# CloudResolvingClimateModeling/sp-coupler

Measured on AMD Instinct MI355X. Metric: SP column-exchanges/sec (GCM<->LES forcing+tendency), higher is better.
Workload: dtype f64

## Files before the change

sp_coupler_amd/csrc/spc_hip.hip:

```cpp
#include <hip/hip_runtime.h>
#include <stdint.h>
#include <stdio.h>
#include <stdlib.h>
#include <string.h>

#include <initializer_list>
#include <type_traits>
#include <unordered_map>

#include "spc.h"

#pragma clang fp contract(off)

#include "spc_pow_coefs.h"
__constant__ double spc_pow_coef_table[21] = {SPC_POW_COEFS};
#define SPC_POW_TABLE spc_pow_coef_table

#ifndef SPC_MUTANT
#define SPC_MUTANT 0
#endif
#define SPC_MUT(n, mutated, original) (SPC_MUTANT == (n) ? (mutated) : (original))

namespace {

// ... 157 lines not shown
template <typename T> struct Bracket {
    int j;
    int mode;
    T x, x0, x1;
};

template <typename T> __device__ __forceinline__ Bracket<T> bracket(const T *xp, int n, int p2, T x)
{
    Bracket<T> b;
    b.x = x;
    if (n == 1) { b.mode = 1; b.j = 0; b.x0 = b.x1 = x; return b; }
    if (x != x) { b.mode = 2; b.j = 0; b.x0 = b.x1 = x; return b; }
    const int j = upper_count(xp, n, p2, x) - 1;
    if (j < 0) { b.mode = 1; b.j = 0; b.x0 = b.x1 = x; return b; }
    if (j >= n - 1) { b.mode = 1; b.j = n - 1; b.x0 = b.x1 = x; return b; }
    b.j = j;
    b.x0 = xp[j];
    b.x1 = xp[j + 1];
    b.mode = (b.x0 == x) ? 1 : 0;
    return b;
}

template <typename T> __device__ __forceinline__ T interp_at(const Bracket<T> &b, const T *fp)
{
    if (b.mode == 2) return b.x;
    if (b.mode == 1) return fp[b.j];
    return lerp_np(b.x, b.x0, b.x1, fp[b.j], fp[b.j + 1]);
}

template <typename T> struct Br {
    int j0, j1;
    bool take, nanx;
    T x, x0, x1;
};

template <typename T> __device__ __forceinline__ Br<T> bracket2(const T *xp, int n, int p2, T x)
{
    Br<T> b;
    const int j = upper_count(xp, n, p2, x) - 1;
    const bool below = j < 0, above = j >= n - 1;
    const int jmax = n >= 2 ? n - 2 : 0;
    const int jc = j < 0 ? 0 : (j > jmax ? jmax : j);
    const T x0 = xp[jc], x1 = xp[jc + 1 < n ? jc + 1 : n - 1];
    b.take = (n == 1) | below | above | (x0 == x);
    b.nanx = (x != x) & (n != 1);
    b.j0 = above ? n - 1 : jc;
    b.j1 = b.take ? b.j0 : jc + 1;
    b.x = x;
    b.x0 = b.take ? T(0) : x0;
    b.x1 = b.take ? T(1) : x1;
    return b;
}

template <int NF, typename T> __device__ __forceinline__ void interp_fields(const Br<T> &b, const T (&f0)[NF], const T (&f1)[NF], T (&r)[NF])
{
    const T t0 = b.x - b.x0;
    const Divisor<T> dx(b.x1 - b.x0);
    T slope[NF];
    bool any_nan = false;
#pragma unroll
    for (int k = 0; k < NF; ++k) {
        slope[k] = dx.div(f1[k] - f0[k]);
        r[k] = slope[k] * t0 + f0[k];
        any_nan |= (r[k] != r[k]);
    }
    if (any_nan & !b.take & !b.nanx) {
        const T t1 = b.x - b.x1;
#pragma unroll
        for (int k = 0; k < NF; ++k) {
            if (r[k] != r[k]) {
                T q = slope[k] * t1 + f1[k];
                if (q != q && f0[k] == f1[k]) q = f0[k];
                r[k] = q;
            }
        }
    }
#pragma unroll
    for (int k = 0; k < NF; ++k) r[k] = b.nanx ? b.x : (b.take ? f0[k] : r[k]);
}

struct DimsP {
    int64_t n_cols, pitchG, pitchGh, pitchL;
    int nG, nL, cb, p2G, p2L, shared_grid, xcd_remap;
};

struct Empty {};

template <typename T> struct FwdOpt {
    const T *rain, *rain_last;
    T *u, *v, *thl, *qt, *ps, *Zf, *Zh, *rainrate;
    const T *Z0M, *Z0H, *QLflux, *QIflux, *SHflux, *TSflux;
    T *z0m, *z0h, *wthl, *wqt;
};

template <typename T, bool FULL> struct FwdP {
    DimsP d;
    const T *U, *V, *Tm, *SH, *QL, *QI, *Pf, *Ph, *Zgfull, *Zghalf, *zf, *zh;
    const T *u_d, *v_d, *thl_d, *qt_d, *ql_d, *ps_d;
    T factor, dt;
    T *f_u, *f_v, *f_thl, *f_qt, *f_ql, *ql_ref, *f_ps;
    int32_t *idx;
    typename std::conditional<FULL, FwdOpt<T>, Empty>::type o;
};

template <typename T> using FwdFull = FwdP<T, true>;

template <typename T> struct BwdP {
    DimsP d;
    const T *Tm, *SH, *QL, *QI, *U, *V, *A, *Zf, *Zgfull, *Zghalf, *zf;
    const T *t_d, *qt_d, *ql_d, *ql_ice_d, *u_d, *v_d, *A_prof;
    const T *zh, *Zh, *rhobf_d;
    T factor, dt;
    T *f_T, *f_SH, *f_QL, *f_QI, *f_U, *f_V, *f_A;
    int32_t *start_index;
};

template <typename T> struct DiagP {
    DimsP d;
    const T *Tm, *SH, *QL, *QI, *Pf, *Zgfull, *Zghalf, *zf, *thl_d, *ql_d, *ql_ice_d;
    T *Tv, *THL, *QT, *Zf, *Zh, *pf, *t, *ql_water;
};

extern __shared__ __align__(16) unsigned char spc_smem[];

__device__ __forceinline__ unsigned slab_index(int remap)
{
    if (remap) {
        const unsigned b = blockIdx.x, nb = gridDim.x, x = b & 7u, j = b >> 3, q = nb >> 3, r = nb & 7u;
        return x * q + (x < r ? x : r) + j;
    }
    return blockIdx.x;
}

#ifdef SPC_STAMPS
__device__ unsigned long long *g_stamps = nullptr;
#define STAMP(i)                                                                     \
    do {                                                                             \
        if (threadIdx.x == 0 && g_stamps && (SPC_STAMPS == 1 || (i) == 0 || (i) == 5)) {  \
            asm volatile("s_waitcnt vmcnt(0) lgkmcnt(0)" ::: "memory");              \
            g_stamps[(size_t)blockIdx.x * 8 + (i)] = wall_clock64();                 \
        }                                                                            \
    } while (0)
#else
#define STAMP(i) do { } while (0)
#endif

template <typename T> struct LesIn {
    T h, ud, vd, thld, qtd, qld;
};

template <typename P, typename T = decltype(+*P().zf)>
__device__ __forceinline__ LesIn<T> load_les(const P &p, int l, int64_t o)
{
    LesIn<T> r;
    r.h = p.d.shared_grid ? ldg(&p.zf[l]) : ldg(&p.zf[o]);
    r.ud = ldg(&p.u_d[o]); r.vd = ldg(&p.v_d[o]); r.thld = ldg(&p.thl_d[o]); r.qtd = ldg(&p.qt_d[o]); r.qld = ldg(&p.ql_d[o]);
    return r;
}

constexpr int cfloor_pow2(int n) { int p = 1; while (p * 2 <= n) p *= 2; return p; }

template <typename T, bool FULL, int NG, int NL, int WT, int BLK = BLOCK, bool PRE = true>
__global__ __launch_bounds__(BLK) void k_forward(const FwdP<T, FULL> p)
{
    const DimsP &d = p.d;
#define OPT(f) (*(decltype(FwdOpt<T>::f) const volatile __attribute__((address_space(4))) *)( \
// ... 142 lines not shown
                f0[k] = s[(k + 1) * nG + b.j0];
                f1[k] = s[(k + 1) * nG + b.j1];
            }
            interp_fields<5>(b, f0, f1, r);
            const T thl = r[0], qt = r[1], ql = r[2], u = r[3], v = r[4];
            stg<WT>(&p.f_u[o], ddt.div(p.factor * (u - SPC_MUT(2, in.vd, in.ud))));
            stg<WT>(&p.f_v[o], ddt.div(p.factor * (v - SPC_MUT(2, in.ud, in.vd))));
            stg<WT>(&p.f_thl[o], ddt.div(p.factor * (thl - in.thld)));
            stg<WT>(&p.f_qt[o], ddt.div(p.factor * (qt - in.qtd)));
            stg<WT>(&p.f_ql[o], ddt.div(p.factor * (ql - in.qld)));
            stg<WT>(&p.ql_ref[o], ql);
            if constexpr (FULL) {
                if (OPT(u)) OPT(u)[o] = u;
                if (OPT(v)) OPT(v)[o] = v;
                if (OPT(thl)) OPT(thl)[o] = thl;
                if (OPT(qt)) OPT(qt)[o] = qt;
            }
        } else {
            const int ei = e - n2, c = ei / nG, m = ei - c * nG;
            const int64_t col = col0 + c, gh = col * pitchGh;
            const T zgh = (PRE && e == tid) ? pre_zgh : ldg(&p.Zghalf[gh + (nG - 1 - m)]);
            const T zs = (PRE && e == tid) ? pre_zs : ldg(&p.Zghalf[gh + nG]);
            const T Zh_k = div_grav(zgh - zs);
            const T *const zh = d.shared_grid ? lzh : lzh + (size_t)c * nL;
            p.idx[col * pitchG + m] = SPC_MUT(5, ss_left_pos(zh, nL, Zh_k), ss_right(zh, nL, Zh_k));
        }
    }
    STAMP(4);

    if constexpr (FULL) {
        if (OPT(Zh)) {
            for (int e = tid; e < ncol * (nG + 1); e += BLK) {
                const int c = e / (nG + 1), k = e - c * (nG + 1);
                const int64_t gh = (col0 + c) * pitchGh;
                OPT(Zh)[gh + k] = div_grav(ldg(&p.Zghalf[gh + k]) - ldg(&p.Zghalf[gh + nG]));
            }
        }
    }
    STAMP(5);
#undef OPT
}

template <typename T>
__global__ __launch_bounds__(BLOCK) void k_cloud_idx(const DimsP d, const T *zh_, const T *Zh_, int32_t *idx)
{
    const int nG = d.nG, nL = d.nL, cb = d.cb, tid = threadIdx.x;
    const int64_t col0 = (int64_t)slab_index(d.xcd_remap) * cb;
    const int ncol = (int)((d.n_cols - col0) < cb ? (d.n_cols - col0) : cb);
    T *const lzh = reinterpret_cast<T *>(spc_smem);
    const int nz = d.shared_grid ? nL : ncol * nL;
    for (int e = tid; e < nz; e += BLOCK) {
        const int c = e / nL, l = e - c * nL;
        lzh[e] = d.shared_grid ? zh_[e] : zh_[(col0 + c) * d.pitchL + l];
    }
    __syncthreads();
    for (int e = tid; e < ncol * nG; e += BLOCK) {
        const int c = e / nG, m = e - c * nG;
        const int64_t col = col0 + c;
        const T *const zh = d.shared_grid ? lzh : lzh + (size_t)c * nL;
        idx[col * d.pitchG + m] = ss_right(zh, nL, Zh_[col * d.pitchGh + (nG - 1 - m)]);
    }
}

template <typename T> struct GcmIn {
    T tt, sh, ql, qi, u, v, a, a_d;
};

template <typename T> __device__ __forceinline__ GcmIn<T> load_gcm(const BwdP<T> &p, int64_t g, int64_t g_rev)
{
    GcmIn<T> r;
    r.tt = ldg(&p.Tm[g]); r.sh = ldg(&p.SH[g]); r.ql = ldg(&p.QL[g]); r.qi = ldg(&p.QI[g]); r.u = ldg(&p.U[g]); r.v = ldg(&p.V[g]); r.a = ldg(&p.A[g]);
    r.a_d = ldg(&p.A_prof[g_rev]);
    return r;
}

template <typename T, int NG, int NL, int WT, int BLK = BLOCK, bool PRE = true> __global__ __launch_bounds__(BLK) void k_backward(const BwdP<T> p)
{
    const DimsP &d = p.d;
    const int nG = NG ? NG : d.nG, nL = NL ? NL : d.nL, cb = d.cb, tid = threadIdx.x;
    const int64_t pitchG = NG ? NG : d.pitchG, pitchGh = NG ? NG + 1 : d.pitchGh, pitchL = NL ? NL : d.pitchL;
    const int p2L = NL ? cfloor_pow2(NL ? NL : 1) : d.p2L;
    const int64_t col0 = (int64_t)slab_index(d.xcd_remap) * cb;
    const int ncol = (int)((d.n_cols - col0) < cb ? (d.n_cols - col0) : cb);
    const size_t per_col = (size_t)6 * nL + nG;
    T *const lds = reinterpret_cast<T *>(spc_smem);
    T *const lh = lds + (size_t)cb * per_col;
    const int n1 = ncol * nG;
    STAMP(0);

    struct Stage { T t, qt, ql, qi, u, v, h; };
    auto load_stage = [&](int64_t o) {
        Stage r;
        r.t = ldg(&p.t_d[o]); r.qt = ldg(&p.qt_d[o]); r.ql = ldg(&p.ql_d[o]); r.qi = ldg(&p.ql_ice_d[o]);
        r.u = ldg(&p.u_d[o]); r.v = ldg(&p.v_d[o]);
        r.h = d.shared_grid ? T(0) : ldg(&p.zf[o]);
        return r;
    };
    auto load_zf = [&](int64_t col, int64_t g) {
        return p.Zf ? p.Zf[g] : div_grav(ldg(&p.Zgfull[g]) - ldg(&p.Zghalf[col * pitchGh + nG]));
    };
    const int n2 = ncol * nL;
    Stage st0 = {};
    T zf0 = T(0), hs0 = T(0);
    if (tid < n2) {
        const int c = tid / nL, l = tid - c * nL;
        st0 = load_stage((col0 + c) * pitchL + l);
    }
    if (tid < n1) {
        const int c = tid / nG, k = tid - c * nG;
        zf0 = load_zf(col0 + c, (col0 + c) * pitchG + k);
    }
    if (d.shared_grid && tid < nL) hs0 = ldg(&p.zf[tid]);
    GcmIn<T> pre = {};
    if (PRE && tid < n1) {
        const int c = tid / nG, k = tid - c * nG;
        const int64_t cg = (col0 + c) * pitchG;
        pre = load_gcm(p, cg + k, SPC_MUT(9, (col0 + ((c ^ 1) < ncol ? (c ^ 1) : c)) * pitchG, cg) + (nG - 1 - k));
    }
    STAMP(1);

    constexpr int UF = sizeof(T) == 4 ? 2 : 1;
    for (int e0 = tid; e0 < n2; e0 += UF * BLK) {
        Stage st[UF];
#pragma unroll
        for (int u = 0; u < UF; ++u) {
            const int e = e0 + u * BLK;
            if (e < n2) {
                const int c = e / nL, l = e - c * nL;
                st[u] = (e == tid) ? st0 : load_stage((col0 + c) * pitchL + l);
            }
        }
#pragma unroll
        for (int u = 0; u < UF; ++u) {
            const int e = e0 + u * BLK;
            if (e < n2) {
                const int c = e / nL, l = e - c * nL;
                T *const s = lds + (size_t)c * per_col + l;
                s[0] = st[u].t;
                s[nL] = st[u].qt;
                s[2 * nL] = st[u].ql;
                s[3 * nL] = st[u].qi;
                s[4 * nL] = st[u].u;
                s[5 * nL] = st[u].v;
                if (!d.shared_grid) lh[e] = st[u].h;
            }
        }
    }
    if (d.shared_grid)
        for (int e = tid; e < nL; e += BLK) lh[e] = (e == tid) ? hs0 : ldg(&p.zf[e]);
    for (int e = tid; e < n1; e += BLK) {
        const int c = e / nG, k = e - c * nG;
        const int64_t col = col0 + c;
        lds[(size_t)c * per_col + 6 * nL + k] = (e == tid) ? zf0 : load_zf(col, col * pitchG + k);
    }
    STAMP(2);
    __syncthreads();
    STAMP(3);

    const Divisor<T> ddt(p.dt);
    auto gcm_item = [&](int e, const GcmIn<T> &in) {
        const int c = e / nG, k = e - c * nG;
        const int64_t col = col0 + c, cg = col * pitchG, g = cg + k;
        const T *const s = lds + (size_t)c * per_col;
        const T *const h = d.shared_grid ? lh : lh + (size_t)c * nL;
        const T *const Zf = s + 6 * nL;
        const T x = Zf[k];
        const int start_index = ss_left_neg(Zf, nG, h[nL - 1]);
        const Bracket<T> b = bracket(h, nL, p2L, x);
        T t_i, qt_i, ql_i, qlw_i, qli_i, u_i, v_i;
        if (b.mode == 0) {
            const int j = b.j;
            const T ql0 = s[2 * nL + j], ql1 = s[2 * nL + j + 1], qi0 = s[3 * nL + j], qi1 = s[3 * nL + j + 1];
            const Divisor<T> dx(b.x1 - b.x0);
            t_i = lerp_np(x, b.x0, b.x1, s[j], s[j + 1], dx);
            qt_i = lerp_np(x, b.x0, b.x1, s[nL + j], s[nL + j + 1], dx);
            ql_i = lerp_np(x, b.x0, b.x1, ql0, ql1, dx);
            qlw_i = lerp_np(x, b.x0, b.x1, ql0 - qi0, ql1 - qi1, dx);
            qli_i = lerp_np(x, b.x0, b.x1, qi0, qi1, dx);
            u_i = lerp_np(x, b.x0, b.x1, s[4 * nL + j], s[4 * nL + j + 1], dx);
            v_i = lerp_np(x, b.x0, b.x1, s[5 * nL + j], s[5 * nL + j + 1], dx);
        } else if (b.mode == 1) {
            const int j = b.j;
            t_i = s[j];
            qt_i = s[nL + j];
            ql_i = s[2 * nL + j];
            qli_i = s[3 * nL + j];
            qlw_i = ql_i - qli_i;
            u_i = s[4 * nL + j];
            v_i = s[5 * nL + j];
        } else {
            t_i = qt_i = ql_i = qlw_i = qli_i = u_i = v_i = x;
        }
        T f_T = ddt.div(p.factor * SPC_MUT(24, in.tt - t_i, t_i - in.tt));
        T f_SH = ddt.div(p.factor * (SPC_MUT(13, qt_i, qt_i - ql_i) - in.sh));
        T f_QL = ddt.div(p.factor * (SPC_MUT(3, ql_i, qlw_i) - in.ql));
        T f_QI = ddt.div(p.factor * (qli_i - in.qi));
        T f_U = ddt.div(p.factor * (SPC_MUT(22, v_i, u_i) - in.u));
        T f_V = ddt.div(p.factor * (v_i - in.v));
        T f_A = ddt.div(p.factor * (in.a_d - in.a));
        if (SPC_MUT(4, k <= start_index, k < start_index)) {
            const T zero = T(0);
            f_T *= zero; f_SH *= zero; f_QL *= zero; f_QI *= zero; f_U *= zero; f_V *= zero; f_A *= zero;
        }
        stg<WT>(&p.f_T[g], f_T);
        stg<WT>(&p.f_SH[g], f_SH);
        stg<WT>(&p.f_QL[g], f_QL);
        stg<WT>(&p.f_QI[g], f_QI);
        stg<WT>(&p.f_U[g], f_U);
        stg<WT>(&p.f_V[g], f_V);
        stg<WT>(&p.f_A[g], f_A);
        if (p.start_index && k == 0) p.start_index[col] = start_index;
    };
    for (int e0 = tid; e0 < n1; e0 += UF * BLK) {
        GcmIn<T> in[UF];
#pragma unroll
        for (int u = 0; u < UF; ++u) {
            const int e = e0 + u * BLK;
            if (e < n1) {
                const int c = e / nG, k = e - c * nG;
                const int64_t cg = (col0 + c) * pitchG;
                in[u] = (PRE && e == tid) ? pre
                                          : load_gcm(p, cg + k, SPC_MUT(9, (col0 + ((c ^ 1) < ncol ? (c ^ 1) : c)) * pitchG, cg) + (nG - 1 - k));
            }
        }
#pragma unroll
        for (int u = 0; u < UF; ++u)
            if (e0 + u * BLK < n1) gcm_item(e0 + u * BLK, in[u]);
    }
    STAMP(4);
    STAMP(5);
}

#include "spc_f32v.hpp"
#include "spc_vnudge.hpp"
#include "spc_vnudge2.hpp"

template <typename T> __device__ __forceinline__ int scan_cell(const T *z, int n, T a)
{
    int lo = 1, hi = n - 1;
    while (lo < hi) {
        const int mid = lo + ((hi - lo) >> 1);
        if (z[mid] < a) lo = mid + 1; else hi = mid;
    }
    return lo - 1;
}

__host__ __device__ inline int su_pad(int p2) { return 2 * p2 + 2; }

template <int SL, typename T, typename Pred> __device__ __forceinline__ const T *su_seek(const T *row, int p2, const Pred &adv)
{
    const T *p = row;
    if constexpr (SL > 0) {
#pragma unroll
        for (int s = 1 << (SL - 1); s > 0; s >>= 1) {
            const T *const nx = p + s;
            p = adv(p[s - 1]) ? nx : p;
        }
    } else {
        for (int s = p2; s > 0; s >>= 1) {
            const T *const nx = p + s;
            p = adv(p[s - 1]) ? nx : p;
        }
    }
    return p;
}

template <int SL, typename T, typename Pred> __device__ __forceinline__ int su_count(const T *row, int p2, const Pred &adv)
{
    return (int)(((unsigned)(size_t)su_seek<SL>(row, p2, adv) - (unsigned)(size_t)row) / (unsigned)sizeof(T));
}

#include "spc_k4.hpp"
// ... 124 lines not shown
    thread_local int cache[64] = {0};
    int dev = 0;
    if (hipGetDevice(&dev) != hipSuccess) {
        (void)hipGetLastError();
        return 256;
    }
    if (dev >= 0 && dev < 64 && cache[dev]) return cache[dev];
    int n = 0;
    if (hipDeviceGetAttribute(&n, hipDeviceAttributeMultiprocessorCount, dev) != hipSuccess || n <= 0) {
        (void)hipGetLastError();
        n = 256;
    }
    if (dev >= 0 && dev < 64) cache[dev] = n;
    return n;
}

template <typename KernelT> int blocks_per_cu(KernelT kernel, size_t smem)
{
    thread_local std::unordered_map<uint64_t, int> cache;
    const uint64_t key = (uint64_t)(uintptr_t)kernel * 1000003u + smem;
    auto it = cache.find(key);
    if (it != cache.end()) return it->second;
    int nb = 0;
    if (hipOccupancyMaxActiveBlocksPerMultiprocessor(&nb, kernel, BLOCK, smem) != hipSuccess || nb <= 0) {
        (void)hipGetLastError();
        const size_t by_lds = smem ? (size_t)(160 * 1024) / smem : 8;
        nb = (int)(by_lds < 4 ? by_lds : 4);
    }
    if (nb > 8) nb = 8;
    cache[key] = nb;
    return nb;
}

template <typename KernelT> int pick_cb(const spc_dims *d, int pass, bool with_idx, size_t esize, KernelT kernel)
{
    size_t per_col, fixed;
    lds_elems(d, pass, with_idx, &per_col, &fixed, esize);
    int cb = d->cols_per_block;
    if (cb > 0) {
        while (cb > 1 && (per_col * cb + fixed) * esize > (size_t)MAX_LDS_BYTES) --cb;
        return cb;
    }
    int nb[4] = {0, 0, 0, 0};
    const int64_t cus = device_cus();
    for (int i = 0; i < 4; ++i) {
        cb = 1 << i;
        const size_t smem = (per_col * cb + fixed) * esize;
        if (cb > 1 && smem > (size_t)MAX_LDS_BYTES) continue;
        nb[i] = blocks_per_cu(kernel, smem);
        if (cb <= 4 && (d->n_cols + cb - 1) / cb <= cus * nb[i]) return cb;
    }
    if (pass == 4 && nb[1] * 2 > nb[0] && (d->n_cols + 1) / 2 >= 2 * cus * nb[1]) return 2;
    int best = 1, best_nb = -1;
    for (int i = (pass == 1 && esize == 4) ? 1 : 3; i >= 0; --i) {
        cb = 1 << i;
        const int64_t rounds_x_cus = nb[i] ? (d->n_cols + cb - 1) / cb / nb[i] : 0;
        const bool enough = rounds_x_cus >= (cb == 8 ? 8 : 2) * cus;
        if (nb[i] > best_nb && (enough || i == 0)) { best_nb = nb[i]; best = cb; }
    }
    return best;
}

int small_batch(int64_t bytes_written, int limit_mib = 32)
{
    return bytes_written <= (int64_t)limit_mib * 1024 * 1024 ? 1 : 0;
}

int geometry_id(const spc_dims *d)
{
    if (d->pitchG != d->nG || d->pitchGh != d->nG + 1 || d->pitchL != d->nL) return 0;
    if (d->nG == 91 && d->nL == 160) return 1;
    if (d->nG == 137 && d->nL == 512) return 2;
    if (d->nG == 19 && d->nL == 160) return 3;
    return 0;
}

DimsP make_dims(const spc_dims *d, int cb)
{
    DimsP p;
    p.n_cols = d->n_cols; p.pitchG = d->pitchG; p.pitchGh = d->pitchGh; p.pitchL = d->pitchL;
    p.nG = d->nG; p.nL = d->nL; p.cb = cb; p.p2G = floor_pow2(d->nG); p.p2L = floor_pow2(d->nL);
    p.shared_grid = d->les_grid_shared != 0;
    p.xcd_remap = cb <= 2;
    return p;
}

template <typename KernelT> int ensure_lds(KernelT kernel, size_t smem, const char *what)
{
    if (smem <= (size_t)MAX_LDS_BYTES) return SPC_OK;
    if (smem > (size_t)HARD_LDS_BYTES)
        return fail(SPC_ERR_UNSUPPORTED, "%s needs %lld B of LDS per workgroup (gfx950 has %lld)", what, (long long)smem, HARD_LDS_BYTES);
    if (hipFuncSetAttribute(reinterpret_cast<const void *>(kernel), hipFuncAttributeMaxDynamicSharedMemorySize, (int)smem) != hipSuccess) {
        (void)hipGetLastError();
        return fail(SPC_ERR_UNSUPPORTED, "%s: cannot raise the dynamic LDS limit to %lld B", what, (long long)smem);
    }
    return SPC_OK;
}

int launch_status(const char *what)
{
    const hipError_t e = hipGetLastError();
    if (e == hipSuccess) return SPC_OK;
    snprintf(g_err, sizeof(g_err), "%s: %s", what, hipGetErrorString(e));
    return SPC_ERR_LAUNCH;
}

#define REQUIRE(ptr, name) \
    if (!(ptr)) return fail(SPC_ERR_INVALID_ARGUMENT, "required pointer %s is NULL", name)

int small_block(const spc_dims *d, int items_per_col)
{
    const int64_t cus = device_cus();
    if (d->cols_per_block != 0 || items_per_col > BLOCK || d->n_cols <= cus || d->n_cols > 4 * cus) return 0;
    const int sb = env_int("SPC_SMALL_BLOCK", 1);
    if (!sb) return 0;
    if (sb == 2 || sb == 4) return sb;
    return d->n_cols <= 2 * cus ? 2 : 4;
}

struct Choice {
    const char *kernel;
    int elem, full, idx, geo, wt, blk, pre, cb;
    int vec = 0;
    unsigned grid;
    size_t smem;
};

constexpr int GEO_NG[4] = {0, 91, 137, 19}, GEO_NL[4] = {0, 160, 512, 160};

template <typename T> using KLean = void (*)(const FwdP<T, false>);
template <typename T> using KFull = void (*)(const FwdP<T, true>);
template <typename T> using KBwd = void (*)(const BwdP<T>);

#define SPC_FWD_ROW(FULL_, WT_, BLK_, PRE_)                                                                          \
    {k_forward<T, FULL_, 0, 0, WT_, BLK_, PRE_>, k_forward<T, FULL_, 91, 160, WT_, BLK_, PRE_>,                      \
     k_forward<T, FULL_, 137, 512, WT_, BLK_, PRE_>, k_forward<T, FULL_, 19, 160, WT_, BLK_, PRE_>}
#define SPC_FWD_ROW_BIG(BLK_)                                                                                        \
    {k_forward<T, false, 0, 0, 1, BLK_, true>, k_forward<T, false, 91, 160, 1, BLK_, true>, nullptr,                 \
     k_forward<T, false, 19, 160, 1, BLK_, true>}

template <typename T> KLean<T> fwd_lean_kernel(int geo, int wt, int blk, int pre)
{
    static const KLean<T> k256[2][2][4] = {{SPC_FWD_ROW(false, 0, BLOCK, false), SPC_FWD_ROW(false, 1, BLOCK, false)},
                                           {SPC_FWD_ROW(false, 0, BLOCK, true), SPC_FWD_ROW(false, 1, BLOCK, true)}};
    static const KLean<T> k512[4] = SPC_FWD_ROW_BIG(512), k1024[4] = SPC_FWD_ROW_BIG(1024);
    if (blk == BLOCK) return k256[pre][wt][geo];
    if (!wt || !pre) return nullptr;
    return blk == 512 ? k512[geo] : (blk == 1024 ? k1024[geo] : nullptr);
}

template <typename T> KFull<T> fwd_full_kernel(int geo, int pre)
{
    static const KFull<T> k[2][4] = {SPC_FWD_ROW(true, 0, BLOCK, false), SPC_FWD_ROW(true, 0, BLOCK, true)};
    return k[pre][geo];
}
#undef SPC_FWD_ROW
#undef SPC_FWD_ROW_BIG

template <typename T> int choose_fwd(const spc_dims *d, bool with_idx, bool full, Choice *c)
{
    c->kernel = "k_forward"; c->elem = (int)sizeof(T); c->full = full; c->idx = with_idx;
    c->geo = geometry_id(d);
    c->wt = full ? 0 : small_batch(d->n_cols * (int64_t)((6 * d->nL + 1) * sizeof(T) + (with_idx ? d->nG * 4 : 0)));
    const int sb = (full || !c->wt) ? 0 : small_block(d, d->nL + (with_idx ? d->nG : 0));
    const int pre_env = env_int("SPC_K1_PRE", -1);
    c->pre = (sb || (pre_env >= 0 ? pre_env != 0 : d->n_cols <= 4 * (int64_t)device_cus())) ? 1 : 0;
    c->blk = sb ? BLOCK * sb : BLOCK;
    if (full)
        c->cb = pick_cb(d, 0, with_idx, sizeof(T), fwd_full_kernel<T>(c->geo, c->pre));
    else
        c->cb = sb ? sb : pick_cb(d, 0, with_idx, sizeof(T), fwd_lean_kernel<T>(c->geo, 0, BLOCK, c->pre));
    size_t per_col, fixed;
    lds_elems(d, 0, with_idx, &per_col, &fixed);
    c->smem = (per_col * c->cb + fixed) * sizeof(T);
    c->grid = (unsigned)((d->n_cols + c->cb - 1) / c->cb);
    c->vec = std::is_same<T, float>::value && c->geo != 0 && !full && !sb && !c->pre && c->cb % 2 == 0 && env_int("SPC_F32_VEC", 1);
    return SPC_OK;
}

inline KLean<float> fwd_vec_kernel(int geo, int wt)
{
    static const KLean<float> k[2][4] = {{nullptr, k_forward_f32v<91, 160, 0>, k_forward_f32v<137, 512, 0>, k_forward_f32v<19, 160, 0>},
                                         {nullptr, k_forward_f32v<91, 160, 1>, k_forward_f32v<137, 512, 1>, k_forward_f32v<19, 160, 1>}};
    return k[wt ? 1 : 0][geo];
}
inline bool aligned8(std::initializer_list<const void *> ptrs)
{
    for (const void *q : ptrs) if ((uintptr_t)q & 7u) return false;
    return true;
}

template <typename T> int forward_impl(const spc_dims *d, const spc_forward_args *a, void *stream)
{
    int rc = validate(d);
    if (rc) return rc;
    if (!a) return fail(SPC_ERR_INVALID_ARGUMENT, "%sargs is NULL");
    if (d->n_cols == 0) return SPC_OK;
    REQUIRE(a->U, "U"); REQUIRE(a->V, "V"); REQUIRE(a->T, "T"); REQUIRE(a->SH, "SH"); REQUIRE(a->QL, "QL");
    REQUIRE(a->QI, "QI"); REQUIRE(a->Pf, "Pf"); REQUIRE(a->Ph, "Ph"); REQUIRE(a->Zgfull, "Zgfull");
    REQUIRE(a->Zghalf, "Zghalf"); REQUIRE(a->zf, "zf"); REQUIRE(a->u_d, "u_d"); REQUIRE(a->v_d, "v_d");
    REQUIRE(a->thl_d, "thl_d"); REQUIRE(a->qt_d, "qt_d"); REQUIRE(a->ql_d, "ql_d"); REQUIRE(a->ps_d, "ps_d");
    REQUIRE(a->f_u, "f_u"); REQUIRE(a->f_v, "f_v"); REQUIRE(a->f_thl, "f_thl"); REQUIRE(a->f_qt, "f_qt");
    REQUIRE(a->f_ql, "f_ql"); REQUIRE(a->ql_ref, "ql_ref"); REQUIRE(a->f_ps, "f_ps");
    if (a->idx && !a->zh) return fail(SPC_ERR_INVALID_ARGUMENT, "%sidx requested but zh is NULL");
    if (a->rainrate && (!a->rain || !a->rain_last))
        return fail(SPC_ERR_INVALID_ARGUMENT, "%srainrate requested but rain / rain_last is NULL");
// ... 48 lines not shown
    int rc = validate(d);
    if (rc) return rc;
    if (d->n_cols == 0) return SPC_OK;
    REQUIRE(zh, "zh"); REQUIRE(Zh, "Zh"); REQUIRE(idx, "idx");
    const int cb = pick_cb(d, 2, true, sizeof(T), k_cloud_idx<T>);
    size_t per_col, fixed;
    lds_elems(d, 2, true, &per_col, &fixed);
    const size_t smem = (per_col * cb + fixed) * sizeof(T);
    if ((rc = ensure_lds(k_cloud_idx<T>, smem, "cloud_indices"))) return rc;
    const unsigned grid = (unsigned)((d->n_cols + cb - 1) / cb);
    hipLaunchKernelGGL(k_cloud_idx<T>, dim3(grid), dim3(BLOCK), smem, (hipStream_t)stream, make_dims(d, cb),
                       (const T *)zh, (const T *)Zh, idx);
    return launch_status("k_cloud_idx");
}

#define SPC_BWD_ROW(WT_, BLK_, PRE_)                                                                                 \
    {k_backward<T, 0, 0, WT_, BLK_, PRE_>, k_backward<T, 91, 160, WT_, BLK_, PRE_>, k_backward<T, 137, 512, WT_, BLK_, PRE_>, \
     k_backward<T, 19, 160, WT_, BLK_, PRE_>}
#define SPC_BWD_ROW_BIG(BLK_)                                                                                        \
    {k_backward<T, 0, 0, 1, BLK_, true>, k_backward<T, 91, 160, 1, BLK_, true>, nullptr, k_backward<T, 19, 160, 1, BLK_, true>}

template <typename T> KBwd<T> bwd_kernel(int geo, int wt, int blk, int pre)
{
    static const KBwd<T> k256[2][2][4] = {{SPC_BWD_ROW(0, BLOCK, false), SPC_BWD_ROW(1, BLOCK, false)},
                                          {SPC_BWD_ROW(0, BLOCK, true), SPC_BWD_ROW(1, BLOCK, true)}};
    static const KBwd<T> k512[4] = SPC_BWD_ROW_BIG(512), k1024[4] = SPC_BWD_ROW_BIG(1024);
    if (blk == BLOCK) return k256[pre][wt][geo];
    if (!wt || !pre) return nullptr;
    return blk == 512 ? k512[geo] : (blk == 1024 ? k1024[geo] : nullptr);
}
#undef SPC_BWD_ROW
#undef SPC_BWD_ROW_BIG

template <typename T> KBwd<T> cons_kernel(int geo, int pd, int cb)
{
    static const KBwd<T> k3[4][2] = {{nullptr, nullptr},
                                     {k_backward_cons3<T, 91, 160, 1>, k_backward_cons3<T, 91, 160, 2>},
                                     {k_backward_cons3<T, 137, 512, 1>, k_backward_cons3<T, 137, 512, 2>},
                                     {k_backward_cons3<T, 19, 160, 1>, k_backward_cons3<T, 19, 160, 2>}};
    if (geo != 0) return k3[geo][cb >= 2 ? 1 : 0];
    if constexpr (std::is_same<T, double>::value) {
        static const KBwd<T> kd[3] = {k_backward_cons2<T, 0, 0, 1>, k_backward_cons2<T, 0, 0, 2>, k_backward_cons2<T, 0, 0, 3>};
        if (pd >= 1 && pd <= 3) return kd[pd - 1];
    }
    return k_backward_cons2<T, 0, 0, -1>;
}

template <typename T> int pick_cb_cons3(const spc_dims *d, int geo)
{
    size_t per_col, fixed;
    lds_elems(d, 4, false, &per_col, &fixed, sizeof(T));
    const size_t smem1 = (per_col + fixed) * sizeof(T), smem2 = (2 * per_col + fixed) * sizeof(T);
    const bool two_fits = smem2 <= (size_t)MAX_LDS_BYTES;
    if (d->cols_per_block > 0) return (d->cols_per_block >= 2 && two_fits) ? 2 : 1;
    const int nb1 = blocks_per_cu(cons_kernel<T>(geo, 0, 1), smem1);
    if (d->n_cols <= (int64_t)device_cus() * nb1 || !two_fits) return 1;
    const int nb2 = blocks_per_cu(cons_kernel<T>(geo, 0, 2), smem2);
    return nb2 * 2 > nb1 ? 2 : 1;
}

int cons_depth(int nL)
{
    if (nL > 1024) return -1;
    static const struct Tab { signed char d[1025]; Tab() { int m = 0; for (int n = 0; n <= 1024; ++n) { if (n >= 129) { const int dn = vn_pw_depth_of(n); if (dn > m) m = dn; } d[n] = (signed char)m; } } } tab;
    const int d = nL < 0 ? 0 : tab.d[nL];
    return d < 1 ? 1 : (d <= 3 ? d : -1);
}

template <typename T> int choose_bwd(const spc_dims *d, bool cons, Choice *c)
{
    c->kernel = cons ? "k_backward_cons2" : "k_backward"; c->elem = (int)sizeof(T); c->full = cons; c->idx = 0;
    c->geo = geometry_id(d);
    c->wt = cons ? 0 : small_batch(d->n_cols * (int64_t)(7 * d->nG * sizeof(T)), 14);
    const int sb = (cons || !c->wt) ? 0 : small_block(d, d->nL > d->nG ? d->nL : d->nG);
    const int64_t cus = device_cus();
    c->pre = (cons || sb || d->n_cols <= 4 * cus || d->n_cols * 256 > 25000 * cus) ? 1 : 0;
    c->blk = sb ? BLOCK * sb : BLOCK;
    c->cb = sb ? sb : (cons ? (c->geo ? pick_cb_cons3<T>(d, c->geo) : pick_cb(d, 4, false, sizeof(T), cons_kernel<T>(0, cons_depth(d->nL), 0)))
                            : pick_cb(d, 1, false, sizeof(T), bwd_kernel<T>(c->geo, 0, BLOCK, c->pre)));
    size_t per_col, fixed;
    lds_elems(d, cons ? 4 : 1, false, &per_col, &fixed, sizeof(T));
    c->smem = (per_col * c->cb + fixed) * sizeof(T);
    c->grid = (unsigned)((d->n_cols + c->cb - 1) / c->cb);
    return SPC_OK;
}

template <typename T> int backward_impl(const spc_dims *d, const spc_backward_args *a, void *stream)
{
    int rc = validate(d);
    if (rc) return rc;
    if (!a) return fail(SPC_ERR_INVALID_ARGUMENT, "%sargs is NULL");
    if (d->n_cols == 0) return SPC_OK;
    REQUIRE(a->T, "T"); REQUIRE(a->SH, "SH"); REQUIRE(a->QL, "QL"); REQUIRE(a->QI, "QI"); REQUIRE(a->U, "U");
    REQUIRE(a->V, "V"); REQUIRE(a->A, "A"); REQUIRE(a->zf, "zf"); REQUIRE(a->t_d, "t_d"); REQUIRE(a->qt_d, "qt_d");
    REQUIRE(a->ql_d, "ql_d"); REQUIRE(a->ql_ice_d, "ql_ice_d"); REQUIRE(a->u_d, "u_d"); REQUIRE(a->v_d, "v_d");
    REQUIRE(a->A_prof, "A_prof"); REQUIRE(a->f_T, "f_T"); REQUIRE(a->f_SH, "f_SH"); REQUIRE(a->f_QL, "f_QL");
    REQUIRE(a->f_QI, "f_QI"); REQUIRE(a->f_U, "f_U"); REQUIRE(a->f_V, "f_V"); REQUIRE(a->f_A, "f_A");
    if (!a->Zf && (!a->Zgfull || !a->Zghalf))
        return fail(SPC_ERR_INVALID_ARGUMENT, "%sneither Zf nor (Zgfull, Zghalf) given");
    const bool cons = a->conservative != 0;
    if (cons) {
        REQUIRE(a->zh, "zh (conservative)"); REQUIRE(a->rhobf_d, "rhobf_d (conservative)");
        if (!a->Zh && !a->Zghalf) return fail(SPC_ERR_INVALID_ARGUMENT, "%sconservative: neither Zh nor Zghalf given");
        if (d->nL < 2) return fail(SPC_ERR_INVALID_ARGUMENT, "%sconservative coarsening needs nL >= 2");
    }
    Choice c;
    if ((rc = choose_bwd<T>(d, cons, &c))) return rc;
    const KBwd<T> kern = cons ? cons_kernel<T>(c.geo, cons_depth(d->nL), c.cb) : bwd_kernel<T>(c.geo, c.wt, c.blk, c.pre);
    if (!kern) return fail(SPC_ERR_UNSUPPORTED, "%sbackward: no kernel instantiated for this launch choice (internal)");
    if ((rc = ensure_lds(kern, c.smem, cons ? "backward (conservative)" : "backward"))) return rc;
    BwdP<T> p;
    p.d = make_dims(d, c.cb);
    p.Tm = (const T *)a->T; CP(SH); CP(QL); CP(QI); CP(U); CP(V); CP(A); CP(Zf); CP(Zgfull); CP(Zghalf); CP(zf);
    CP(t_d); CP(qt_d); CP(ql_d); CP(ql_ice_d); CP(u_d); CP(v_d); CP(A_prof); CP(zh); CP(Zh); CP(rhobf_d);
    p.factor = (T)a->factor; p.dt = (T)a->dt;
    OP(f_T); OP(f_SH); OP(f_QL); OP(f_QI); OP(f_U); OP(f_V); OP(f_A); p.start_index = a->start_index;
    hipLaunchKernelGGL(kern, dim3(c.grid), dim3(c.blk), c.smem, (hipStream_t)stream, p);
    return launch_status(cons ? "k_backward_cons" : "k_backward");
}

template <typename T> using KDiag = void (*)(const DiagP<T>);

template <typename T> KDiag<T> diag_kernel(int geo, int wt)
{
    static const KDiag<T> k[2][4] = {{k_diag<T, 0, 0, 0>, k_diag<T, 91, 160, 0>, k_diag<T, 137, 512, 0>, k_diag<T, 19, 160, 0>},
                                     {k_diag<T, 0, 0, 1>, k_diag<T, 91, 160, 1>, k_diag<T, 137, 512, 1>, k_diag<T, 19, 160, 1>}};
    return k[wt ? 1 : 0][geo];
}

template <typename T> int choose_diag(const spc_dims *d, const spc_diagnostics_args *a, Choice *c)
{
    c->kernel = "k_diag"; c->elem = (int)sizeof(T); c->full = c->idx = 0; c->pre = 0; c->blk = BLOCK;
    c->geo = geometry_id(d);
    const int64_t nGw = !a ? 4 : (a->Tv != nullptr) + (a->THL != nullptr) + (a->QT != nullptr) + (a->Zf != nullptr);
    const int64_t nLw = !a ? 3 : (a->pf != nullptr) + (a->t != nullptr) + (a->ql_water != nullptr);
    const int64_t elems = nGw * d->nG + ((!a || a->Zh) ? d->nG + 1 : 0) + ((!a || a->zf) ? nLw * d->nL : 0);
    c->wt = small_batch(d->n_cols * elems * (int64_t)sizeof(T));
    c->cb = pick_cb(d, 3, false, sizeof(T), diag_kernel<T>(c->geo, 0));
    size_t per_col, fixed;
    lds_elems(d, 3, false, &per_col, &fixed);
    c->smem = (per_col * c->cb + fixed) * sizeof(T);
    c->grid = (unsigned)((d->n_cols + c->cb - 1) / c->cb);
    return SPC_OK;
}

template <typename T> int diag_impl(const spc_dims *d, const spc_diagnostics_args *a, void *stream)
{
    int rc = validate(d);
    if (rc) return rc;
    if (!a) return fail(SPC_ERR_INVALID_ARGUMENT, "%sargs is NULL");
    if (d->n_cols == 0) return SPC_OK;
    REQUIRE(a->T, "T"); REQUIRE(a->SH, "SH"); REQUIRE(a->QL, "QL"); REQUIRE(a->QI, "QI"); REQUIRE(a->Pf, "Pf");
    REQUIRE(a->Zgfull, "Zgfull"); REQUIRE(a->Zghalf, "Zghalf");
    if ((a->pf || a->t || a->ql_water) && !a->zf) return fail(SPC_ERR_INVALID_ARGUMENT, "%sLES diagnostics need zf");
    if (a->t && (!a->thl_d || !a->ql_d)) return fail(SPC_ERR_INVALID_ARGUMENT, "%st needs thl_d and ql_d");
    if (a->ql_water && (!a->ql_d || !a->ql_ice_d)) return fail(SPC_ERR_INVALID_ARGUMENT, "%sql_water needs ql_d and ql_ice_d");
    Choice c;
    if ((rc = choose_diag<T>(d, a, &c))) return rc;
    const KDiag<T> kern = diag_kernel<T>(c.geo, c.wt);
    const int cb = c.cb;
    const size_t smem = c.smem;
    if ((rc = ensure_lds(kern, smem, "diagnostics"))) return rc;
    DiagP<T> p;
    p.d = make_dims(d, cb);
    p.Tm = (const T *)a->T; CP(SH); CP(QL); CP(QI); CP(Pf); CP(Zgfull); CP(Zghalf); CP(zf); CP(thl_d); CP(ql_d); CP(ql_ice_d);
    OP(Tv); OP(THL); OP(QT); OP(Zf); OP(Zh); OP(pf); OP(t); OP(ql_water);
    const unsigned grid = (unsigned)((d->n_cols + cb - 1) / cb);
    hipLaunchKernelGGL(kern, dim3(grid), dim3(BLOCK), smem, (hipStream_t)stream, p);
    return launch_status("k_diag");
}
#undef CP
#undef OP
#undef COP
#undef OOP

template <typename T>
int surface_impl(int64_t n, const void *Ph_s, const void *T_s, const void *QLflux, const void *QIflux,
                        const void *SHflux, const void *TSflux, void *wthl, void *wqt, void *stream)
{
    if (n < 0) return fail(SPC_ERR_INVALID_ARGUMENT, "%ssurface_fluxes: n < 0");
    if (n == 0) return SPC_OK;
    if (!Ph_s || !T_s || !QLflux || !QIflux || !SHflux || !TSflux || !wthl || !wqt)
        return fail(SPC_ERR_INVALID_ARGUMENT, "%ssurface_fluxes: NULL pointer");
    const unsigned grid = (unsigned)((n + BLOCK - 1) / BLOCK < 2048 ? (n + BLOCK - 1) / BLOCK : 2048);
    hipLaunchKernelGGL(k_surface<T>, dim3(grid), dim3(BLOCK), 0, (hipStream_t)stream, n, (const T *)Ph_s, (const T *)T_s,
                       (const T *)QLflux, (const T *)QIflux, (const T *)SHflux, (const T *)TSflux, (T *)wthl, (T *)wqt);
    return launch_status("k_surface");
}

template <typename T> int describe_impl(const spc_dims *d, int pass, int flags, Choice *c)
{
    switch (pass) {
    case 0: return choose_fwd<T>(d, (flags & 1) != 0, (flags & 2) != 0, c);
    case 1: return choose_bwd<T>(d, false, c);
    case 4: return choose_bwd<T>(d, true, c);
    case 3: return choose_diag<T>(d, nullptr, c);
    case 2: {
        c->kernel = "k_cloud_idx"; c->elem = (int)sizeof(T); c->full = c->idx = c->geo = c->wt = c->pre = 0;
        c->blk = BLOCK;
// ... 153 lines not shown

#ifdef SPC_STAMPS
int spc_debug_set_stamps(void *buf)
{
    return hipMemcpyToSymbol(HIP_SYMBOL(g_stamps), &buf, sizeof(buf)) == hipSuccess ? 0 : SPC_ERR_LAUNCH;
}
#endif

int spc_exner_f64(int64_t n, const void *p, void *out, int32_t inv, void *s) { return exner_impl<double>(n, p, out, inv, s); }
int spc_exner_f32(int64_t n, const void *p, void *out, int32_t inv, void *s) { return exner_impl<float>(n, p, out, inv, s); }
int spc_interp_f64(const spc_interp_args *a, void *s) { return interp_impl<double>(a, s); }
int spc_interp_f32(const spc_interp_args *a, void *s) { return interp_impl<float>(a, s); }
int spc_searchsorted_f64(const spc_searchsorted_args *a, void *s) { return searchsorted_impl<double>(a, s); }
int spc_searchsorted_f32(const spc_searchsorted_args *a, void *s) { return searchsorted_impl<float>(a, s); }
int spc_interp_c_f64(const spc_interp_c_args *a, void *s) { return interp_c_impl<double>(a, s); }
int spc_interp_c_f32(const spc_interp_c_args *a, void *s) { return interp_c_impl<float>(a, s); }
int spc_rms_f64(int64_t nr, int64_t n, int64_t pitch, const void *a, void *out, void *s) { return rms_impl<double>(nr, n, pitch, a, out, s); }
int spc_rms_f32(int64_t nr, int64_t n, int64_t pitch, const void *a, void *out, void *s) { return rms_impl<float>(nr, n, pitch, a, out, s); }

int spc_surface_fluxes_f64(int64_t n, const void *Ph_s, const void *T_s, const void *QLflux, const void *QIflux,
                           const void *SHflux, const void *TSflux, void *wthl, void *wqt, void *stream)
{
    return surface_impl<double>(n, Ph_s, T_s, QLflux, QIflux, SHflux, TSflux, wthl, wqt, stream);
}

int spc_surface_fluxes_f32(int64_t n, const void *Ph_s, const void *T_s, const void *QLflux, const void *QIflux,
                           const void *SHflux, const void *TSflux, void *wthl, void *wqt, void *stream)
{
    return surface_impl<float>(n, Ph_s, T_s, QLflux, QIflux, SHflux, TSflux, wthl, wqt, stream);
}

int64_t spc_vnudge_workspace_bytes(int64_t n_cols, int32_t itot, int32_t jtot, int32_t ktot)
{
    return vnudge_workspace_bytes<double>(n_cols, itot, jtot, ktot);
}
int64_t spc_vnudge_workspace_bytes_f32(int64_t n_cols, int32_t itot, int32_t jtot, int32_t ktot)
{
    return vnudge_workspace_bytes<float>(n_cols, itot, jtot, ktot);
}
int spc_variability_nudge_f64(const spc_vnudge_args *a, void *stream) { return vnudge_impl<double>(a, stream); }
int spc_variability_nudge_f32(const spc_vnudge_args *a, void *stream) { return vnudge_impl<float>(a, stream); }

int spc_abi_version(void) { return SPC_ABI_VERSION; }
const char *spc_last_error(void) { return g_err; }

int spc_device_count(void)
{
    int n = 0;
    if (hipGetDeviceCount(&n) != hipSuccess) {
        (void)hipGetLastError();
        return 0;
    }
    return n;
}

int spc_describe_launch(const spc_dims *d, int pass, int flags, int elem_size, char *buf, int buflen)
{
    int rc = validate(d);
    if (rc) return rc;
    if (!buf || buflen < 1) return fail(SPC_ERR_INVALID_ARGUMENT, "%sdescribe_launch: no buffer");
    if (elem_size != 8 && elem_size != 4) return fail(SPC_ERR_INVALID_ARGUMENT, "%sdescribe_launch: elem_size must be 8 or 4");
    Choice c = {};
    rc = elem_size == 8 ? describe_impl<double>(d, pass, flags, &c) : describe_impl<float>(d, pass, flags, &c);
    if (rc) return rc;
    const char *ty = elem_size == 8 ? "f64" : "f32";
    char name[160];
    if (pass == 0 && c.vec)
        snprintf(name, sizeof(name), "k_forward_f32v<%d,%d,wt=%d>", GEO_NG[c.geo], GEO_NL[c.geo], c.wt);
    else if (pass == 0)
        snprintf(name, sizeof(name), "k_forward<%s,%s,%d,%d,wt=%d,blk=%d,pre=%d>", ty, c.full ? "full" : "lean", GEO_NG[c.geo], GEO_NL[c.geo],
                 c.wt, c.blk, c.pre);
    else if (pass == 1)
        snprintf(name, sizeof(name), "k_backward<%s,%d,%d,wt=%d,blk=%d,pre=%d>", ty, GEO_NG[c.geo], GEO_NL[c.geo], c.wt, c.blk, c.pre);
    else if (pass == 4)
        if (c.geo == 0)
            snprintf(name, sizeof(name), "k_backward_cons2<%s,0,0,pd=%d>", ty, elem_size == 8 ? cons_depth(d->nL) : -1);
        else
            snprintf(name, sizeof(name), "k_backward_cons3<%s,%d,%d,cb=%d>", ty, GEO_NG[c.geo], GEO_NL[c.geo], c.cb >= 2 ? 2 : 1);
    else if (pass == 3)
        snprintf(name, sizeof(name), "k_diag<%s,%d,%d,wt=%d>", ty, GEO_NG[c.geo], GEO_NL[c.geo], c.wt);
    else
        snprintf(name, sizeof(name), "%s<%s>", c.kernel, ty);
    const char *form = pass != 0 ? "" : (c.vec ? " form=vec" : (c.pre ? " form=whole" : " form=reach"));
    return snprintf(buf, (size_t)buflen, "%s cb=%d grid=%u block=%d lds=%lld cus=%d%s", name, c.cb, c.grid, c.blk, (long long)c.smem,
                    device_cus(), form);
}

int spc_pick_cols_per_block(const spc_dims *d, int pass)
{
    int rc = validate(d);
    if (rc) return rc;
    Choice c = {};
    rc = describe_impl<double>(d, pass, 1, &c);
    return rc ? rc : c.cb;
}

}
```

Before: 139.6 million.

## Stage backward LES profiles into LDS via direct global-to-LDS DMA

Reorganizes the backward kernel's LDS from per-column interleaved blocks into field-major rows, with the GCM height profile in its own region. For fixed-geometry kernels with 16-byte-aligned inputs, it copies the six LES fields and the height grid straight from global memory into LDS using global_load_lds 16-byte transfers, bypassing registers. The goal is to cut register staging and per-element LDS stores in the load phase. The trade-offs are reliance on contiguous pitch and divisibility assumptions, a correctness dependence on the DMA completing before the barrier, and a separate register fallback path.

```diff
diff --git a/sp_coupler_amd/csrc/spc_hip.hip b/sp_coupler_amd/csrc/spc_hip.hip
--- a/sp_coupler_amd/csrc/spc_hip.hip
+++ b/sp_coupler_amd/csrc/spc_hip.hip
@@ -263,6 +263,7 @@
 struct DimsP {
     int64_t n_cols, pitchG, pitchGh, pitchL;
     int nG, nL, cb, p2G, p2L, shared_grid, xcd_remap;
+    int lds_dma;
 };
 
 struct Empty {};
@@ -571,10 +572,12 @@
     const int p2L = NL ? cfloor_pow2(NL ? NL : 1) : d.p2L;
     const int64_t col0 = (int64_t)slab_index(d.xcd_remap) * cb;
     const int ncol = (int)((d.n_cols - col0) < cb ? (d.n_cols - col0) : cb);
-    const size_t per_col = (size_t)6 * nL + nG;
+    const size_t rowsL = (size_t)cb * nL;
     T *const lds = reinterpret_cast<T *>(spc_smem);
-    T *const lh = lds + (size_t)cb * per_col;
-    const int n1 = ncol * nG;
+    T *const lh = lds + 6 * rowsL;
+    T *const lzf = lh + (d.shared_grid ? (size_t)nL : rowsL);
+    const int n1 = ncol * nG, n2 = ncol * nL;
+    const bool zf_given = p.Zf != nullptr;
     STAMP(0);
 
     struct Stage { T t, qt, ql, qi, u, v, h; };
@@ -585,21 +588,48 @@
         r.h = d.shared_grid ? T(0) : ldg(&p.zf[o]);
         return r;
     };
-    auto load_zf = [&](int64_t col, int64_t g) {
-        return p.Zf ? p.Zf[g] : div_grav(ldg(&p.Zgfull[g]) - ldg(&p.Zghalf[col * pitchGh + nG]));
-    };
-    const int n2 = ncol * nL;
+    const bool dma = NG != 0 && d.lds_dma;
     Stage st0 = {};
-    T zf0 = T(0), hs0 = T(0);
-    if (tid < n2) {
-        const int c = tid / nL, l = tid - c * nL;
-        st0 = load_stage((col0 + c) * pitchL + l);
-    }
+    T hs0 = T(0);
+    if constexpr (NG != 0) {
+        if (dma) {
+            constexpr int E = 16 / (int)sizeof(T);
+            const int lane = tid & 63, nw = BLK / 64;
+            int i = __builtin_amdgcn_readfirstlane(tid >> 6);
+            auto copy_rows = [&](const T *src, T *dst, int np) {
+                const int nins = (np + 63) >> 6;
+                for (; i < nins; i += nw) {
+                    const int q = (i << 6) + lane;
+                    if (q < np)
+                        __builtin_amdgcn_global_load_lds((const void *)(src + (size_t)q * E),
+                                                         (__attribute__((address_space(3))) void *)(dst + ((size_t)i << 6) * E), 16, 0, 0);
+                }
+                i -= nins;
+            };
+            const int64_t o = col0 * nL;
+            copy_rows(p.t_d + o, lds, n2 / E);
+            copy_rows(p.qt_d + o, lds + rowsL, n2 / E);
+            copy_rows(p.ql_d + o, lds + 2 * rowsL, n2 / E);
+            copy_rows(p.ql_ice_d + o, lds + 3 * rowsL, n2 / E);
+            copy_rows(p.u_d + o, lds + 4 * rowsL, n2 / E);
+            copy_rows(p.v_d + o, lds + 5 * rowsL, n2 / E);
+            copy_rows(d.shared_grid ? p.zf : p.zf + o, lh, (d.shared_grid ? nL : n2) / E);
+        }
+    }
+    if (!dma) {
+        if (tid < n2) {
+            const int c = tid / nL, l = tid - c * nL;
+            st0 = load_stage((col0 + c) * pitchL + l);
+        }
+        if (d.shared_grid && tid < nL) hs0 = ldg(&p.zf[tid]);
+    }
+    T za0 = T(0), zb0 = T(0);
     if (tid < n1) {
         const int c = tid / nG, k = tid - c * nG;
-        zf0 = load_zf(col0 + c, (col0 + c) * pitchG + k);
-    }
-    if (d.shared_grid && tid < nL) hs0 = ldg(&p.zf[tid]);
+        const int64_t col = col0 + c, g = col * pitchG + k;
+        za0 = ldg(zf_given ? &p.Zf[g] : &p.Zgfull[g]);
+        zb0 = ldg(zf_given ? &p.Zf[g] : &p.Zghalf[col * pitchGh + nG]);
+    }
     GcmIn<T> pre = {};
     if (PRE && tid < n1) {
         const int c = tid / nG, k = tid - c * nG;
@@ -609,38 +639,40 @@
     STAMP(1);
 
     constexpr int UF = sizeof(T) == 4 ? 2 : 1;
-    for (int e0 = tid; e0 < n2; e0 += UF * BLK) {
-        Stage st[UF];
+    if (!dma) {
+        for (int e0 = tid; e0 < n2; e0 += UF * BLK) {
+            Stage st[UF];
 #pragma unroll
-        for (int u = 0; u < UF; ++u) {
-            const int e = e0 + u * BLK;
-            if (e < n2) {
-                const int c = e / nL, l = e - c * nL;
-                st[u] = (e == tid) ? st0 : load_stage((col0 + c) * pitchL + l);
+            for (int u = 0; u < UF; ++u) {
+                const int e = e0 + u * BLK;
+                if (e < n2) {
+                    const int c = e / nL, l = e - c * nL;
+                    st[u] = (e == tid) ? st0 : load_stage((col0 + c) * pitchL + l);
+                }
             }
-        }
 #pragma unroll
-        for (int u = 0; u < UF; ++u) {
-            const int e = e0 + u * BLK;
-            if (e < n2) {
-                const int c = e / nL, l = e - c * nL;
-                T *const s = lds + (size_t)c * per_col + l;
-                s[0] = st[u].t;
-                s[nL] = st[u].qt;
-                s[2 * nL] = st[u].ql;
-                s[3 * nL] = st[u].qi;
-                s[4 * nL] = st[u].u;
-                s[5 * nL] = st[u].v;
-                if (!d.shared_grid) lh[e] = st[u].h;
+            for (int u = 0; u < UF; ++u) {
+                const int e = e0 + u * BLK;
+                if (e < n2) {
+                    T *const s = lds + e;
+                    s[0] = st[u].t;
+                    s[rowsL] = st[u].qt;
+                    s[2 * rowsL] = st[u].ql;
+                    s[3 * rowsL] = st[u].qi;
+                    s[4 * rowsL] = st[u].u;
+                    s[5 * rowsL] = st[u].v;
+                    if (!d.shared_grid) lh[e] = st[u].h;
+                }
             }
         }
-    }
-    if (d.shared_grid)
-        for (int e = tid; e < nL; e += BLK) lh[e] = (e == tid) ? hs0 : ldg(&p.zf[e]);
-    for (int e = tid; e < n1; e += BLK) {
+        if (d.shared_grid)
+            for (int e = tid; e < nL; e += BLK) lh[e] = (e == tid) ? hs0 : ldg(&p.zf[e]);
+    }
+    if (tid < n1) lzf[tid] = zf_given ? za0 : div_grav(za0 - zb0);
+    for (int e = tid + BLK; e < n1; e += BLK) {
         const int c = e / nG, k = e - c * nG;
-        const int64_t col = col0 + c;
-        lds[(size_t)c * per_col + 6 * nL + k] = (e == tid) ? zf0 : load_zf(col, col * pitchG + k);
+        const int64_t col = col0 + c, g = col * pitchG + k;
+        lzf[e] = zf_given ? ldg(&p.Zf[g]) : div_grav(ldg(&p.Zgfull[g]) - ldg(&p.Zghalf[col * pitchGh + nG]));
     }
     STAMP(2);
     __syncthreads();
@@ -650,33 +682,33 @@
     auto gcm_item = [&](int e, const GcmIn<T> &in) {
         const int c = e / nG, k = e - c * nG;
         const int64_t col = col0 + c, cg = col * pitchG, g = cg + k;
-        const T *const s = lds + (size_t)c * per_col;
+        const T *const s = lds + (size_t)c * nL;
         const T *const h = d.shared_grid ? lh : lh + (size_t)c * nL;
-        const T *const Zf = s + 6 * nL;
+        const T *const Zf = lzf + (size_t)c * nG;
         const T x = Zf[k];
         const int start_index = ss_left_neg(Zf, nG, h[nL - 1]);
         const Bracket<T> b = bracket(h, nL, p2L, x);
         T t_i, qt_i, ql_i, qlw_i, qli_i, u_i, v_i;
         if (b.mode == 0) {
             const int j = b.j;
-            const T ql0 = s[2 * nL + j], ql1 = s[2 * nL + j + 1], qi0 = s[3 * nL + j], qi1 = s[3 * nL + j + 1];
+            const T ql0 = s[2 * rowsL + j], ql1 = s[2 * rowsL + j + 1], qi0 = s[3 * rowsL + j], qi1 = s[3 * rowsL + j + 1];
             const Divisor<T> dx(b.x1 - b.x0);
             t_i = lerp_np(x, b.x0, b.x1, s[j], s[j + 1], dx);
-            qt_i = lerp_np(x, b.x0, b.x1, s[nL + j], s[nL + j + 1], dx);
+            qt_i = lerp_np(x, b.x0, b.x1, s[rowsL + j], s[rowsL + j + 1], dx);
             ql_i = lerp_np(x, b.x0, b.x1, ql0, ql1, dx);
             qlw_i = lerp_np(x, b.x0, b.x1, ql0 - qi0, ql1 - qi1, dx);
             qli_i = lerp_np(x, b.x0, b.x1, qi0, qi1, dx);
-            u_i = lerp_np(x, b.x0, b.x1, s[4 * nL + j], s[4 * nL + j + 1], dx);
-            v_i = lerp_np(x, b.x0, b.x1, s[5 * nL + j], s[5 * nL + j + 1], dx);
+            u_i = lerp_np(x, b.x0, b.x1, s[4 * rowsL + j], s[4 * rowsL + j + 1], dx);
+            v_i = lerp_np(x, b.x0, b.x1, s[5 * rowsL + j], s[5 * rowsL + j + 1], dx);
         } else if (b.mode == 1) {
             const int j = b.j;
             t_i = s[j];
-            qt_i = s[nL + j];
-            ql_i = s[2 * nL + j];
-            qli_i = s[3 * nL + j];
+            qt_i = s[rowsL + j];
+            ql_i = s[2 * rowsL + j];
+            qli_i = s[3 * rowsL + j];
             qlw_i = ql_i - qli_i;
-            u_i = s[4 * nL + j];
-            v_i = s[5 * nL + j];
+            u_i = s[4 * rowsL + j];
+            v_i = s[5 * rowsL + j];
         } else {
             t_i = qt_i = ql_i = qlw_i = qli_i = u_i = v_i = x;
         }
@@ -967,6 +999,7 @@
     p.nG = d->nG; p.nL = d->nL; p.cb = cb; p.p2G = floor_pow2(d->nG); p.p2L = floor_pow2(d->nL);
     p.shared_grid = d->les_grid_shared != 0;
     p.xcd_remap = cb <= 2;
+    p.lds_dma = 0;
     return p;
 }
 
@@ -1007,6 +1040,7 @@
     const char *kernel;
     int elem, full, idx, geo, wt, blk, pre, cb;
     int vec = 0;
+    int dma = 0;
     unsigned grid;
     size_t smem;
 };
@@ -1221,7 +1255,14 @@
     lds_elems(d, cons ? 4 : 1, false, &per_col, &fixed, sizeof(T));
     c->smem = (per_col * c->cb + fixed) * sizeof(T);
     c->grid = (unsigned)((d->n_cols + c->cb - 1) / c->cb);
+    c->dma = !cons && c->geo != 0;
     return SPC_OK;
+}
+
+inline bool aligned16(std::initializer_list<const void *> ptrs)
+{
+    for (const void *q : ptrs) if ((uintptr_t)q & 15u) return false;
+    return true;
 }
 
 template <typename T> int backward_impl(const spc_dims *d, const spc_backward_args *a, void *stream)
@@ -1254,6 +1295,7 @@
     CP(t_d); CP(qt_d); CP(ql_d); CP(ql_ice_d); CP(u_d); CP(v_d); CP(A_prof); CP(zh); CP(Zh); CP(rhobf_d);
     p.factor = (T)a->factor; p.dt = (T)a->dt;
     OP(f_T); OP(f_SH); OP(f_QL); OP(f_QI); OP(f_U); OP(f_V); OP(f_A); p.start_index = a->start_index;
+    p.d.lds_dma = c.dma && aligned16({a->t_d, a->qt_d, a->ql_d, a->ql_ice_d, a->u_d, a->v_d, a->zf});
     hipLaunchKernelGGL(kern, dim3(c.grid), dim3(c.blk), c.smem, (hipStream_t)stream, p);
     return launch_status(cons ? "k_backward_cons" : "k_backward");
 }
@@ -1573,8 +1615,9 @@
     else
         snprintf(name, sizeof(name), "%s<%s>", c.kernel, ty);
     const char *form = pass != 0 ? "" : (c.vec ? " form=vec" : (c.pre ? " form=whole" : " form=reach"));
-    return snprintf(buf, (size_t)buflen, "%s cb=%d grid=%u block=%d lds=%lld cus=%d%s", name, c.cb, c.grid, c.blk, (long long)c.smem,
-                    device_cus(), form);
+    const char *stage = pass != 1 ? "" : (c.dma ? " stage=dma" : " stage=regs");
+    return snprintf(buf, (size_t)buflen, "%s cb=%d grid=%u block=%d lds=%lld cus=%d%s%s", name, c.cb, c.grid, c.blk, (long long)c.smem,
+                    device_cus(), form, stage);
 }
 
 int spc_pick_cols_per_block(const spc_dims *d, int pass)
```

After: 140.4 million, median of 6. Within noise of the previous version (+0.6%).
